# V-Sense/LFBM5D

Hardware: AMD Instinct MI355X
Metric: SAI-megapixels/sec (HT+Wiener, sigma=25) (higher is better)
Workload: dtype f32; 1 GPU; lf17x17x512x512_sigma25; light_field=17x17x512x512x3, asw=1, color_space=opp, noise=MT19937 seed 1 (utilities.cpp:176-183), window_lanes=2, spatial_bands=1, parallelism=single GPU

## Files before the change

### lfbm5d_amd/core.py

```python
import ctypes as C
import os
import subprocess

from typing import NamedTuple, Optional

import numpy as np

_HERE = os.path.dirname(os.path.abspath(__file__))

YUV, YCBCR, OPP, RGB, ID, DCT, SADCT, BIOR, HADAMARD, HAAR = range(10)
ROWMAJOR, COLMAJOR = 11, 12
TAU = {"id": ID, "dct": DCT, "sadct": SADCT, "bior": BIOR, "hw": HADAMARD, "haar": HAAR}
COLOR_SPACE = {"yuv": YUV, "ycbcr": YCBCR, "opp": OPP, "rgb": RGB}
UNIQUE_ID_BYTES = 128


class LfBm5dError(RuntimeError):
    pass


class Params(C.Structure):
    _fields_ = [("sigma", C.c_float), ("lambda_", C.c_float), ("N", C.c_uint), ("nSim", C.c_uint),
                ("nDisp", C.c_uint), ("k", C.c_uint), ("p", C.c_uint), ("useSD", C.c_uint),
                ("tau_2D", C.c_uint), ("tau_4D", C.c_uint), ("tau_5D", C.c_uint),
# ... 232 lines not shown
    out = (C.c_void_p * len(arrays))()
    for i, a in enumerate(arrays):
        if a is None or not mask[i]:
            continue
        if not (isinstance(a, np.ndarray) and a.dtype == np.float32 and a.flags.c_contiguous):
            raise LfBm5dError("per-SAI host buffers must be contiguous float32 numpy arrays")
        out[i] = a.ctypes.data
    return out


OPTION_ENV = ("LFBM5D_LANES", "LFBM5D_EMULATE_WORLD", "LFBM5D_MAX_WINDOWS", "LFBM5D_FUSED", "LFBM5D_STEP_SHARDING",
              "LFBM5D_DATA_DRIVEN_SCHEDULE", "LFBM5D_HOST_BLOCKING", "LFBM5D_BAND_MB", "LFBM5D_BM3D_LANES", "LFBM5D_SCAN_LDS_CAP",
              "LFBM5D_FORCE_REDO", "LFBM5D_SPATIAL_BANDS", "LFBM5D_BAND_HALO", "LFBM5D_SCAN_V1", "LFBM5D_SCAN_ANY", "LFBM5D_SCAN_FULL_TABLES", "LFBM5D_DCT8W_V2",
              "LFBM5D_GROUP_GENERIC", "LFBM5D_NO_SA_KERNELS", "LFBM5D_NO_SLAB_KERNEL", "LFBM5D_WIDE_NOSPLIT", "LFBM5D_AGG_64BIT",
              "LFBM5D_AGG_SCALAR_SCAN", "LFBM5D_SUBSET_LIST_HOST", "LFBM5D_SUBSET_SCAN_V1", "LFBM5D_FILT_GROUP_MAJOR",
              "LFBM5D_HT_REF_ORDER")


class Context:

    def __init__(self, device=0):
        self._L = lib()
        h = C.c_void_p()
        if self._L.lfbm5d_create(C.byref(h), int(device)) != 0:
            raise LfBm5dError(self._L.lfbm5d_last_error(None).decode())
        self._handle = h
        self._env_seen = {k: os.environ.get(k) for k in OPTION_ENV}
        self.device = int(device)

    @property
    def _h(self):
# ... 275 lines not shown
```

### lfbm5d_amd/csrc/lfbm5d_api.hip

```cpp
#include "lfbm5d_graph.h"

using namespace lfbm5d_host;
using lfbm5d::plan::search_window;
using lfbm5d::plan::plan_windows;

namespace { std::string g_create_error; }

extern "C" {

int lfbm5d_device_count(void) {
    int n = 0;
    if (hipGetDeviceCount(&n) != hipSuccess) return 0;
    return n;
}

int lfbm5d_create(lfbm5d_ctx** out, int device) {
    if (!out) return 1;
    *out = nullptr;
    int n = 0;
    hipError_t e = hipGetDeviceCount(&n);
    if (e != hipSuccess || n <= 0) {
        g_create_error = "no HIP device available (liblfbm5d_hip has no CPU fallback)";
        return 1;
    }
// ... 14 lines not shown
int lfbm5d_get_option(lfbm5d_ctx* c, const char* key, char* value, unsigned long long size) {
    if (!c || !key || !value || size == 0) return 1;
    std::string v;
    if (!option_get(c->opt_store, key, v)) return fail(c, std::string("unknown option: ") + key);
    std::snprintf(value, (size_t)size, "%s", v.c_str());
    return 0;
}

void lfbm5d_destroy(lfbm5d_ctx* c) {
    if (!c) return;
    (void)hipSetDevice(c->device);
    for (lfbm5d_ctx* x : c->lanes) lfbm5d_destroy(x);
    c->lanes.clear();
    if (c->h_counts) (void)hipHostFree(c->h_counts);
    if (c->stream) (void)hipStreamSynchronize(c->stream);
    for (lfbm5d_ctx::IpcPeer& P : c->ipc_peers) for (void* q : P.ptr) if (q) (void)hipIpcCloseMemHandle(q);
    c->ipc_flags.release(); c->ipc_out.release(); c->pristine.release(); c->pristine_b.release();
    if (c->io_in) (void)hipStreamDestroy(c->io_in);
    if (c->io_out) (void)hipStreamDestroy(c->io_out);
    if (c->team_comm2) ncclCommDestroy(c->team_comm2);
    if (c->team_comm) ncclCommDestroy(c->team_comm);
    if (c->comm2) ncclCommDestroy(c->comm2);
    if (c->comm) ncclCommDestroy(c->comm);
    for (int i = 0; i < 2; i++) if (c->cs[i]) (void)hipStreamDestroy(c->cs[i]);
    for (GeomCache& g : c->gc) { g.refs.release(); g.rslot.release(); g.tb.release(); g.scan_wgs.release(); }
    DevBuf* bufs[] = {&c->est, &c->g_num2, &c->g_den2, &c->n2, &c->e_basic, &c->refmap, &c->scores, &c->tables, &c->self_idx, &c->self_cnt, &c->best,
                      &c->t_noisy, &c->t_basic, &c->t_tnum, &c->t_tden, &c->und_num, &c->und_den, &c->sub_flags, &c->sub_cnt, &c->shape, &c->filt, &c->wgt, &c->aggpos, &c->gpos, &c->gofs, &c->gok, &c->sa_list, &c->gshape, &c->band_noisy, &c->band_basic, &c->band_out, &c->band_src, &c->band_pack, &c->band_gather, &c->counters, &c->small, &c->t_num, &c->t_den, &c->d_mask, &c->g_num, &c->g_den, &c->w_noisy,
                      &c->w_basic, &c->w_num, &c->w_den, &c->h2d_noisy, &c->h2d_basic, &c->h2d_out, &c->d_own, &c->gscratch, &c->scan_lcol};
    for (DevBuf* b : bufs) b->release();
    c->noise.sai.release(); c->noise.part.release(); c->noise.cells.release(); c->noise.m.release(); c->noise.pool.release();
    for (hipEvent_t e : c->ev_pool) (void)hipEventDestroy(e);
    if (c->h_small) (void)hipHostFree(c->h_small);
    if (c->stream) (void)hipStreamDestroy(c->stream);
    delete c;
}

const char* lfbm5d_last_error(const lfbm5d_ctx* c) { return c ? c->err.c_str() : g_create_error.c_str(); }
void lfbm5d_reset_stats(lfbm5d_ctx* c) { if (c) std::memset(&c->stats, 0, sizeof(c->stats)); }
void lfbm5d_get_stats(const lfbm5d_ctx* c, lfbm5d_stats* out) { if (c && out) *out = c->stats; }
void* lfbm5d_stream(lfbm5d_ctx* c) { return c ? (void*)c->stream : nullptr; }

void lfbm5d_shard_rows(unsigned n_rows, int rank, int world, unsigned* begin, unsigned* end) {
    if (world < 1) world = 1;
    if (rank < 0) rank = 0;
    *begin = (unsigned)(((unsigned long long)n_rows * (unsigned)rank) / (unsigned)world);
    *end = (unsigned)(((unsigned long long)n_rows * (unsigned)(rank + 1)) / (unsigned)world);
}
// ... 540 lines not shown
```

### lfbm5d_amd/csrc/lfbm5d_ctx.h

```cpp
#ifndef LFBM5D_CTX_H
#define LFBM5D_CTX_H

#include "../../include/lfbm5d.h"
#include "lfbm5d_kernels.h"
#include "lfbm5d_plan.h"
#include "lfbm5d_options.h"

#include <rccl/rccl.h>

#include <algorithm>
#include <chrono>
#include <cmath>
#include <fstream>
#include <thread>
#include <unistd.h>
#include <cstdio>
#include <cstdlib>
#include <cstring>
#include <string>
#include <vector>


namespace lfbm5d_host {

// ... 12 lines not shown
        if (p) { hipError_t e = hipFree(p); p = nullptr; cap = 0; if (e != hipSuccess) return e; }
        hipError_t e = hipMalloc(&p, bytes);
        if (e == hipSuccess) cap = bytes;
        return e;
    }
    void release() { if (p) (void)hipFree(p); p = nullptr; cap = 0; }
    template <class T> T* as() const { return reinterpret_cast<T*>(p); }
};

struct PassEvents { hipEvent_t e[5]; bool comm; };

struct GeomCache {
    DevBuf refs, rslot, tb, scan_wgs;
    std::vector<Scan2Wg> scan_plan; unsigned scan_key[8] = {0, 0, 0, 0, 0, 0, 0, 0}; size_t scan_lds = 0;
    unsigned scan_nwg_slot = 0; int scan_version = 0;
    std::vector<unsigned> last_refs_host;
    unsigned grid_key[5] = {0, 0, 0, 0, 0};
    unsigned rslot_key[5] = {0, 0, 0, 0, 0};
    unsigned tb_key[3] = {0, 0, 0};
    unsigned n_ref_rows = 0, n_ref_cols = 0;
};

}

using lfbm5d_host::DevBuf; using lfbm5d_host::PassEvents; using lfbm5d_host::GeomCache; using lfbm5d::Options;


constexpr int kDefaultLanes = 2;
constexpr size_t kEstLead = 64;

struct HostIO {
    float* const* noisy = nullptr;
    float* const* basic = nullptr;
    float* const* out = nullptr;
};

struct lfbm5d_ctx {
    int device = 0;
    hipStream_t stream = nullptr;
    std::string err;
    int rank = 0, world = 1;
    int tiles = 1;
    ncclComm_t comm = nullptr;
    ncclComm_t comm2 = nullptr;
    hipStream_t cs[2] = {nullptr, nullptr};
    int pass_rank = 0, pass_world = 1;
    bool pass_reduce = false;
    std::vector<unsigned> last_windows;
    lfbm5d_stats stats;
    DevBuf t_noisy, t_basic, t_tnum, t_tden, und_num, und_den;
    DevBuf scan_lcol;
    DevBuf sub_flags, sub_cnt;
    int last_scan_version = 0;
    GeomCache gc[2]; int gslot = 0;
// ... 69 lines not shown
```

### lfbm5d_amd/csrc/lfbm5d_graph.hip

```cpp
#include "lfbm5d_graph.h"

namespace lfbm5d_host {

using plan::search_window;
using plan::plan_windows;

int io_upload_all(lfbm5d_ctx* c, const HostIO* io, const unsigned* h_mask, unsigned asize, size_t img, float* d_noisy, float* d_basic_in) {
    for (unsigned st = 0; st < asize; st++) {
        if (!h_mask[st]) continue;
        HIPCK(c, hipMemcpyAsync(d_noisy + (size_t)st * img, io->noisy[st], img * sizeof(float), hipMemcpyHostToDevice, c->stream));
        if (d_basic_in) HIPCK(c, hipMemcpyAsync(d_basic_in + (size_t)st * img, io->basic[st], img * sizeof(float), hipMemcpyHostToDevice, c->stream));
    }
    HIPCK(c, hipStreamSynchronize(c->stream));
    return 0;
}
int io_download_all(lfbm5d_ctx* c, const HostIO* io, const unsigned* h_mask, unsigned asize, size_t img, const float* d_noisy,
                    const float* d_basic, const float* d_out) {
    for (unsigned st = 0; st < asize; st++) {
        if (!h_mask[st]) continue;
        HIPCK(c, hipMemcpyAsync(io->noisy[st], d_noisy + (size_t)st * img, img * sizeof(float), hipMemcpyDeviceToHost, c->stream));
        if (d_basic) HIPCK(c, hipMemcpyAsync(io->basic[st], d_basic + (size_t)st * img, img * sizeof(float), hipMemcpyDeviceToHost, c->stream));
        if (d_out) HIPCK(c, hipMemcpyAsync(io->out[st], d_out + (size_t)st * img, img * sizeof(float), hipMemcpyDeviceToHost, c->stream));
    }
    HIPCK(c, hipStreamSynchronize(c->stream));
// ... 295 lines not shown
            const unsigned cst_w = ang_major == LFBM5D_ROWMAJOR ? (unsigned)cs_w * g.asw + (unsigned)ct_w : (unsigned)cs_w + (unsigned)ct_w * g.asw;
            std::vector<unsigned> mask_w(g.Aw, 0), proc_w(g.Aw, 0);
            SaiList wl; wl.n = g.Aw;
            for (unsigned si = 0; si < g.asw; si++)
                for (unsigned ti = 0; ti < g.asw; ti++) {
                    const unsigned Ss = si + (unsigned)mins, T = ti + (unsigned)mint;
                    const unsigned st = ang_major == LFBM5D_ROWMAJOR ? Ss * awidth + T : Ss + T * aheight;
                    const unsigned slot = ang_major == LFBM5D_ROWMAJOR ? si * g.asw + ti : si + ti * g.asw;
                    mask_w[slot] = h_mask[st];
                    wl.st[slot] = h_mask[st] ? st : 0xffffffffu;
                    if (h_mask[st]) win_bits[n].set(slot);
                    proc_w[slot] = !h_mask[st];
                }
            const bool wien = J.step[sl] == 2;
            HIPCK(c, Lw.x->est.reserve((kEstLead + g.Aw * (size_t)g.wb * g.hb + 256) * sizeof(float)));
            HIPCK(c, launch_window_begin(ls, J.noisy[sl], wien ? S->basic : nullptr, S->g_num[sl], S->g_den[sl], img, Lw.w_noisy, Lw.w_basic, Lw.w_num,
                                         Lw.w_den, Lw.x->est.as<float>() + kEstLead, g.imgb, wl, W, H, C, g.nHW, Lw.d_small));
            lfbm5d_params Pw = *J.P[sl];
            Pw.tau_4D = nd.tau4;
            Lw.x->gslot = sl;
            Lw.x->est_ready = true;
            const int prc = pass_impl(Lw.x, J.step[sl], &Pw, g.asw, g.asw, g.wb, g.hb, C, Lw.w_noisy, wien ? Lw.w_basic : nullptr, Lw.w_num, Lw.w_den,
                                      mask_w.data(), proc_w.data(), cst_w, cst_w);
            Lw.x->gslot = 0;
            if (prc) { if (Lw.x != c) c->err = Lw.x->err; return 1; }
            HIPCK(c, launch_window_end(ls, S->g_num[sl], S->g_den[sl], img, Lw.w_num, Lw.w_den, g.imgb, wl, W, H, C, g.nHW, J.P[sl]->k, Lw.d_small));
            HIPCK(c, hipMemcpyAsync(c->h_counts + (size_t)n * kWinCounters, Lw.d_small, kWinCounters * sizeof(unsigned), hipMemcpyDeviceToHost, ls));
            if (!nd.fin.empty()) {
                SaiList fl; fl.n = 0;
                for (unsigned st : nd.fin) fl.st[fl.n++] = st;
                const bool colour = C == 3 && J.P[0]->color_space != LFBM5D_RGB;
                HIPCK(c, launch_finalize_multi(ls, S->g_num[0], S->g_den[0], J.noisy[0], S->basic, img, fl, J.P[0]->color_space, W * H, colour ? 1 : 0));
// ... 240 lines not shown
```

### lfbm5d_amd/csrc/lfbm5d_kernels.h

```cpp
#ifndef LFBM5D_KERNELS_H
#define LFBM5D_KERNELS_H

#include <hip/hip_runtime.h>
#include <vector>

#include "lfbm5d_options.h"

constexpr int kFiltStoreAux = 2;
constexpr int kFiltLoadAux = 0;

#if defined(__HIPCC__)
typedef float filt_v4f __attribute__((ext_vector_type(4)));
typedef float filt_v2f __attribute__((ext_vector_type(2)));
__device__ __forceinline__ void filt_put(float* p, const float v) { *p = v; }
__device__ __forceinline__ void filt_put2(filt_v2f* p, const filt_v2f v) { *p = v; }
__device__ __forceinline__ void filt_put4(filt_v4f* p, const filt_v4f v) { *p = v; }
__device__ __forceinline__ void filt_put4(float4* p, const float4 v) { *p = v; }
__device__ __forceinline__ void filt_put4_nt(filt_v4f* p, const filt_v4f v) { __builtin_nontemporal_store(v, p); }
#endif

namespace lfbm5d {

constexpr int kMaxK = 32;
constexpr int kMaxA = 49;
// ... 193 lines not shown
struct SaiList { unsigned st[kBigA]; unsigned n; };
hipError_t launch_finalize_multi(hipStream_t s, const float* num, const float* den, const float* sub, float* basic, size_t sai_stride,
                                 const SaiList& L, unsigned cs, unsigned n_px, int colour);
hipError_t launch_output_multi(hipStream_t s, const float* num, const float* den, const float* sub, float* out, float* basic,
                               const float* noisy_src, float* noisy_dst, size_t sai_stride, const SaiList& L, unsigned cs, unsigned n_px,
                               int colour);
hipError_t launch_ipc_set(hipStream_t s, unsigned* p, unsigned v);
hipError_t launch_ipc_wait(hipStream_t s, const unsigned* p, unsigned want, unsigned* err, double timeout_s);
hipError_t launch_symetrize_multi(hipStream_t s, const float* src, size_t src_stride, float* dst, size_t dst_stride,
                                  const SaiList& L, unsigned W, unsigned H, unsigned C, unsigned N);
hipError_t launch_unsymetrize_multi(hipStream_t s, float* dst, size_t dst_stride, const float* src, size_t src_stride,
                                    const SaiList& L, unsigned W, unsigned H, unsigned C, unsigned N);
constexpr unsigned kWinCounters = 32;
hipError_t launch_window_begin(hipStream_t s, const float* noisy, const float* basic, const float* num, const float* den, size_t lf_stride,
                               float* w_noisy, float* w_basic, float* w_num, float* w_den, float* est, size_t w_stride, const SaiList& L,
                               unsigned W, unsigned H, unsigned C, unsigned N, unsigned* zero);
hipError_t launch_window_end(hipStream_t s, float* num, float* den, size_t lf_stride, const float* w_num, const float* w_den, size_t w_stride,
                             const SaiList& L, unsigned W, unsigned H, unsigned C, unsigned N, unsigned k, unsigned* count);
hipError_t launch_estimate_multi(hipStream_t s, const float* num, const float* den, const float* sub, float* est,
                                 size_t plane, unsigned C, unsigned A, const SaiMask& mask_bits);
hipError_t launch_copy_rect(hipStream_t s, float* dst, size_t dst_stride, unsigned dW, unsigned dH, unsigned dx0, unsigned dy0,
                            const float* src, size_t src_stride, unsigned sW, unsigned sH, unsigned sx0, unsigned sy0,
                            unsigned w, unsigned h, unsigned C, unsigned n_slots, const SaiMask& mask_bits);
hipError_t launch_copy_rows(hipStream_t s, const float* src, unsigned src_H, unsigned src_row0, float* dst, unsigned dst_H, unsigned dst_row0,
                            unsigned n_rows, unsigned W, unsigned planes);
hipError_t launch_fill_f32(hipStream_t s, float* p, float v, size_t n);
hipError_t launch_fill_i32(hipStream_t s, int* p, int v, size_t n);
hipError_t launch_add(hipStream_t s, float* dst, const float* src, size_t n);
hipError_t launch_count_zeros(hipStream_t s, const float* den, size_t seg, unsigned n_seg,
                              unsigned* counts);
hipError_t launch_count_denoised(hipStream_t s, const float* den, size_t sai_stride, unsigned n_slots, const SaiMask& mask_bits,
                                 unsigned W, unsigned H, unsigned C, unsigned N, unsigned k, unsigned* count);
hipError_t launch_refmap(hipStream_t s, const unsigned* refs, unsigned n_refs, int* refmap);
hipError_t launch_subset_list(hipStream_t s, const float* den0, unsigned Wb, unsigned k, unsigned nHW, unsigned p, unsigned n_rows,
                              unsigned n_cols, unsigned last_r, unsigned last_c, unsigned char* flags, unsigned* refs, unsigned* count);
hipError_t launch_bm_scan(hipStream_t s, const ScanArgs& a);
int bm_scan_version(const ScanArgs& a);
bool scan2_plan(const ScanArgs& a, std::vector<Scan2Wg>& wgs, size_t* lds_bytes, unsigned* nwg_slot = nullptr);
size_t scan_tables_floats(const ScanArgs& a, int version, unsigned n_slots, unsigned nwg_slot);
unsigned scan2_lcol_stride(const ScanArgs& a);
hipError_t prepare_scan2_kernels();
hipError_t launch_bm_scan2(hipStream_t s, const ScanArgs& a, size_t lds_bytes, bool combined);
hipError_t launch_stereo_argmin3(hipStream_t s, const float* tables, const unsigned* st_of_slot, unsigned n_slots, unsigned nwg_slot,
                                 unsigned W, unsigned H, unsigned k, unsigned nDisp, float thr,
                                 unsigned* best, unsigned char* shape);
hipError_t launch_stereo_argmin2(hipStream_t s, const float* tables, const unsigned* st_of_slot, unsigned n_slots,
                                 unsigned W, unsigned H, unsigned k, unsigned nDisp, float thr,
                                 unsigned* best, unsigned char* shape);
hipError_t launch_self_select(hipStream_t s, const float* scores, const unsigned* refs, unsigned n_refs,
                              unsigned W, unsigned nSim, unsigned N, float thr, unsigned* self_idx,
                              unsigned* self_cnt,
                              unsigned grid_cols = 0, unsigned nHW = 0, unsigned p = 1, unsigned last_r = 0, unsigned last_c = 0);
hipError_t launch_self_trivial(hipStream_t s, const unsigned* refs, unsigned n_refs, unsigned* self_idx,
                               unsigned* self_cnt);
hipError_t launch_stereo_argmin(hipStream_t s, const float* tables, const unsigned* st_of_slot, unsigned n_slots,
                                unsigned W, unsigned H, unsigned k, unsigned nDisp, float thr,
                                unsigned* best, unsigned char* shape);
// ... 9 lines not shown
```

### lfbm5d_amd/csrc/lfbm5d_options.h

```cpp
#ifndef LFBM5D_OPTIONS_H
#define LFBM5D_OPTIONS_H

#include <cstddef>
#include <cstdlib>
#include <cstring>
#include <string>

namespace lfbm5d {

enum : unsigned {
    kOptScanV1 = 1u << 0,
    kOptScanAny = 1u << 1,
    kOptScanFullTables = 1u << 2,
    kOptDct8wV2 = 1u << 3,
    kOptGroupGeneric = 1u << 4,
    kOptNoSaKernels = 1u << 5,
    kOptNoSlabKernel = 1u << 6,
    kOptWideNoSplit = 1u << 7,
    kOptAgg64Bit = 1u << 8,
    kOptAggScalarScan = 1u << 9,
    kOptSubsetListHost = 1u << 10,
    kOptSubsetScanV1 = 1u << 11,
    kOptFiltGroupMajor = 1u << 12,
    kOptHtReferenceOrder = 1u << 13,
// ... 1 lines not shown

struct Options {
    int lanes = 2;
    int emulate_world = 0;
    int max_windows = 0;
    int fused = 1;
    int step_sharding = 0;
    int data_driven_schedule = 0;
    int host_blocking = 0;
    int band_mb = 0;
    int bm3d_lanes = 3;
    int scan_lds_cap = 0;
    int force_redo = 0;
    int spatial_bands = 1;
    int band_halo = 0;
    unsigned kernels = 0;
};

struct OptionKey { const char* key; const char* env; int Options::* field; unsigned bit; };

inline const OptionKey* option_keys(size_t* n) {
    static const OptionKey keys[] = {
        {"lanes", "LFBM5D_LANES", &Options::lanes, 0}, {"emulate_world", "LFBM5D_EMULATE_WORLD", &Options::emulate_world, 0},
        {"max_windows", "LFBM5D_MAX_WINDOWS", &Options::max_windows, 0}, {"fused", "LFBM5D_FUSED", &Options::fused, 0},
        {"step_sharding", "LFBM5D_STEP_SHARDING", &Options::step_sharding, 0},
        {"data_driven_schedule", "LFBM5D_DATA_DRIVEN_SCHEDULE", &Options::data_driven_schedule, 0},
        {"host_blocking", "LFBM5D_HOST_BLOCKING", &Options::host_blocking, 0}, {"band_mb", "LFBM5D_BAND_MB", &Options::band_mb, 0},
        {"bm3d_lanes", "LFBM5D_BM3D_LANES", &Options::bm3d_lanes, 0}, {"scan_lds_cap", "LFBM5D_SCAN_LDS_CAP", &Options::scan_lds_cap, 0},
        {"force_redo", "LFBM5D_FORCE_REDO", &Options::force_redo, 0}, {"spatial_bands", "LFBM5D_SPATIAL_BANDS", &Options::spatial_bands, 0},
        {"band_halo", "LFBM5D_BAND_HALO", &Options::band_halo, 0},
        {"scan_v1", "LFBM5D_SCAN_V1", nullptr, kOptScanV1}, {"scan_any", "LFBM5D_SCAN_ANY", nullptr, kOptScanAny},
        {"scan_full_tables", "LFBM5D_SCAN_FULL_TABLES", nullptr, kOptScanFullTables}, {"dct8w_v2", "LFBM5D_DCT8W_V2", nullptr, kOptDct8wV2},
        {"group_generic", "LFBM5D_GROUP_GENERIC", nullptr, kOptGroupGeneric}, {"no_sa_kernels", "LFBM5D_NO_SA_KERNELS", nullptr, kOptNoSaKernels},
        {"no_slab_kernel", "LFBM5D_NO_SLAB_KERNEL", nullptr, kOptNoSlabKernel}, {"wide_nosplit", "LFBM5D_WIDE_NOSPLIT", nullptr, kOptWideNoSplit},
        {"agg_64bit", "LFBM5D_AGG_64BIT", nullptr, kOptAgg64Bit}, {"agg_scalar_scan", "LFBM5D_AGG_SCALAR_SCAN", nullptr, kOptAggScalarScan},
        {"subset_list_host", "LFBM5D_SUBSET_LIST_HOST", nullptr, kOptSubsetListHost}, {"subset_scan_v1", "LFBM5D_SUBSET_SCAN_V1", nullptr, kOptSubsetScanV1},
        {"filt_group_major", "LFBM5D_FILT_GROUP_MAJOR", nullptr, kOptFiltGroupMajor},
        {"ht_reference_order", "LFBM5D_HT_REF_ORDER", nullptr, kOptHtReferenceOrder},
    };
    *n = sizeof(keys) / sizeof(keys[0]);
    return keys;
}

inline bool option_set(Options& o, const char* key, const char* value) {
    size_t n; const OptionKey* keys = option_keys(&n);
// ... 44 lines not shown
```

### lfbm5d_amd/csrc/lfbm5d_pass.hip

```cpp
#include "lfbm5d_ctx.h"

namespace lfbm5d_host {

lfbm5d_ctx* new_ctx(int device, std::string& err) {
    hipError_t e;
    lfbm5d_ctx* c = new lfbm5d_ctx();
    c->device = device;
    std::memset(&c->stats, 0, sizeof(c->stats));
    if ((e = hipStreamCreateWithFlags(&c->stream, hipStreamNonBlocking)) != hipSuccess) { err = hipGetErrorString(e); delete c; return nullptr; }
    if ((e = prepare_group_kernels()) != hipSuccess || (e = prepare_scan2_kernels()) != hipSuccess) { err = std::string("kernel LDS limits: ") + hipGetErrorString(e); (void)hipStreamDestroy(c->stream); delete c; return nullptr; }
    if ((e = hipHostMalloc((void**)&c->h_small, 64 * sizeof(unsigned))) != hipSuccess) { err = hipGetErrorString(e); (void)hipStreamDestroy(c->stream); delete c; return nullptr; }
    return c;
}


hipEvent_t get_event(lfbm5d_ctx* c) {
    if (c->ev_used == c->ev_pool.size()) {
        hipEvent_t e; (void)hipEventCreate(&e); c->ev_pool.push_back(e);
    }
    return c->ev_pool[c->ev_used++];
}

void drain_events(lfbm5d_ctx* c) {
    for (const PassEvents& pe : c->pending) {
        float ms = 0;
        if (hipEventElapsedTime(&ms, pe.e[0], pe.e[1]) == hipSuccess) c->stats.ms_bm += ms;
// ... 119 lines not shown
    if (P->tau_4D != LFBM5D_ID && P->tau_4D != LFBM5D_DCT && P->tau_4D != LFBM5D_SADCT) return fail(c, "bad tau_4D");
    if (P->tau_5D != LFBM5D_HAAR && P->tau_5D != LFBM5D_HADAMARD && P->tau_5D != LFBM5D_DCT) return fail(c, "bad tau_5D");
    if (!is_pow2(P->N) || P->N > (unsigned)kMaxN3) return fail(c, "unsupported: N must be a power of two <= 32");
    if (P->nSim < 1 || P->nDisp < 1 || P->p < 1) return fail(c, "bad search window / step");
    if (P->nSim > 48 || P->nDisp > 24) return fail(c, "unsupported: nSim > 48 or nDisp > 24");
    (void)step;
    return 0;
}

int pass_impl(lfbm5d_ctx* c, int step, const lfbm5d_params* P, unsigned aw, unsigned ah, unsigned Wb,
              unsigned Hb, unsigned C, const float* d_noisy, const float* d_basic, float* d_num,
              float* d_den, const unsigned* h_mask, const unsigned* h_proc, unsigned cst, unsigned pst,
              bool bm3d) {
    const bool est_ready = c->est_ready;
    c->est_ready = false;
    if (validate(c, step, P, aw, ah, C, bm3d)) return 1;
    if (step == 2 && !d_basic) return fail(c, "step 2 needs the basic estimate");
    const unsigned A = aw * ah, k = P->k, k2 = k * k, N = P->N, nHW = P->nSim + P->nDisp;
    const size_t plane = (size_t)Wb * Hb;
    hipStream_t s = c->stream;
    GeomCache& gc = c->gc[c->gslot];
    if (Hb < 2 * nHW + k + 1 || Wb < 2 * nHW + k + 1) return fail(c, "window smaller than the search range");
    if (Hb > 65535 || Wb > 65535) return fail(c, "unsupported: window larger than 65535 pixels a side");

    float sig[3] = {0, 0, 0};
    if (sigma_table(P->sigma, C, P->color_space, sig)) return fail(c, "bad color space");
    const float tauMatch = bm3d ? (step == 1 ? (C == 1 ? 3.f : 1.f) * (sig[0] < 35.0f ? 2500 : 5000)
                                             : (sig[0] < 35.0f ? 400.f : 3500.f))
                                : (C == 1 ? 3.f : 1.f) * (sig[0] < 35.0f ? (step == 1 ? 3000 : 2000) : 5000);
    const float thr = tauMatch * k * k;
// ... 145 lines not shown
        HIPCK(c, hipMemsetAsync(d_den, 0, A * C * plane * sizeof(float), s));
    }

    HIPCK(c, hipEventRecord(pe.e[0], s));
    ScanArgs sa;
    std::memset(&sa, 0, sizeof(sa));
    sa.dbg = d_counters + 4;
    sa.est = est; sa.W = Wb; sa.H = Hb; sa.k = k; sa.pst = pst;
    sa.nSim = P->nSim; sa.nDisp = P->nDisp; sa.nHW = nHW;
    sa.n_ref_rows = gc.n_ref_rows; sa.n_ref_cols = gc.n_ref_cols; sa.p = P->p;
    sa.scores = c->scores.as<float>(); sa.tables = c->tables.as<float>(); sa.rslot = gc.rslot.as<int>(); sa.refmap = (centre || full_scan) ? nullptr : c->refmap.as<int>(); sa.scores_bytes = (unsigned)((size_t)R_sc * NsS * NsS * sizeof(float));
    sa.n_self = N > 1 ? (P->nSim + 1) * NsS : 0;
    sa.n_stereo = n_slots * NsD * NsD;
    for (unsigned i = 0; i < n_slots; i++) sa.st_of_slot[i] = slots[i];
    sa.est_planes = A;
    if (N > 1) HIPCK(c, launch_fill_f32(s, c->scores.as<float>(), 2 * thr, (size_t)R_sc * NsS * NsS));
    sa.opt = c->opt->kernels; sa.lds_cap = (unsigned)std::max(0, c->opt->scan_lds_cap);
    const bool opt_v1 = (sa.opt & (kOptScanV1 | kOptScanAny)) != 0, opt_ft = (sa.opt & kOptScanFullTables) != 0;
    const unsigned skey[8] = {sa.n_self, sa.n_stereo, sa.nSim, sa.nDisp, sa.k, Hb, Wb,
                              1u | ((centre || full_scan) ? 0u : 2u) | (opt_v1 ? 4u : 0u) | (opt_ft ? 8u : 0u) | ((sa.opt & kOptScanAny) ? 16u : 0u)};
    const bool scan_changed = std::memcmp(skey, gc.scan_key, sizeof(skey)) != 0;
    if (scan_changed) gc.scan_version = bm_scan_version(sa);
    const int scan_version = gc.scan_version;
    c->last_scan_version = scan_version;
    if (scan_version == 1) {
        HIPCK(c, c->tables.reserve(std::max<size_t>(1, scan_tables_floats(sa, 1, n_slots, 0)) * sizeof(float)));
        sa.tables = c->tables.as<float>();
    }
    if (scan_version >= 2) {
        if (scan_changed) {
            if (!scan2_plan(sa, gc.scan_plan, &gc.scan_lds, &gc.scan_nwg_slot)) return fail(c, "scan plan");
            HIPCK(c, gc.scan_wgs.reserve(gc.scan_plan.size() * sizeof(Scan2Wg)));
            HIPCK(c, hipMemcpyAsync(gc.scan_wgs.p, gc.scan_plan.data(), gc.scan_plan.size() * sizeof(Scan2Wg), hipMemcpyHostToDevice, s));
            HIPCK(c, hipStreamSynchronize(s));
        }
        sa.wgs = gc.scan_wgs.as<Scan2Wg>(); sa.n_wgs = (unsigned)gc.scan_plan.size();
        sa.lcol_stride = scan2_lcol_stride(sa);
        HIPCK(c, c->scan_lcol.reserve((size_t)(sa.n_self + sa.n_stereo) * sa.lcol_stride * sizeof(float)));
        sa.lcol = c->scan_lcol.as<float>();
        sa.nwg_slot = gc.scan_nwg_slot;
        HIPCK(c, c->tables.reserve(std::max<size_t>(1, scan_tables_floats(sa, scan_version, n_slots, sa.nwg_slot)) * sizeof(float)));
        sa.tables = c->tables.as<float>();
        HIPCK(c, launch_bm_scan2(s, sa, gc.scan_lds, scan_version == 3));
    } else
        HIPCK(c, launch_bm_scan(s, sa));
    std::memcpy(gc.scan_key, skey, sizeof(skey));
    if (N > 1)
        HIPCK(c, launch_self_select(s, c->scores.as<float>(), gc.refs.as<unsigned>(), R, Wb, P->nSim, N, thr,
                                    c->self_idx.as<unsigned>(), c->self_cnt.as<unsigned>(),
                                    full_scan ? gc.n_ref_cols : 0u, nHW, P->p, Hb - k - nHW, Wb - k - nHW));
    else
        HIPCK(c, launch_self_trivial(s, gc.refs.as<unsigned>(), R, c->self_idx.as<unsigned>(), c->self_cnt.as<unsigned>()));
    if (n_slots && scan_version == 3)
        HIPCK(c, launch_stereo_argmin3(s, c->tables.as<float>(), slots, n_slots, sa.nwg_slot, Wb, Hb, k, P->nDisp, thr,
                                       c->best.as<unsigned>(), c->shape.as<unsigned char>()));
    else if (n_slots && scan_version == 2)
        HIPCK(c, launch_stereo_argmin2(s, c->tables.as<float>(), slots, n_slots, Wb, Hb, k, P->nDisp, thr,
                                       c->best.as<unsigned>(), c->shape.as<unsigned char>()));
    else if (n_slots)
        HIPCK(c, launch_stereo_argmin(s, c->tables.as<float>(), slots, n_slots, Wb, Hb, k, P->nDisp, thr,
                                      c->best.as<unsigned>(), c->shape.as<unsigned char>()));
    HIPCK(c, hipEventRecord(pe.e[1], s));

    unsigned ref_begin, n_groups;
    if (centre) {
        unsigned rb = 0, re = gc.n_ref_rows;
        lfbm5d_shard_rows(gc.n_ref_rows, c->pass_rank, c->pass_world, &rb, &re);
        ref_begin = rb * gc.n_ref_cols; n_groups = (re - rb) * gc.n_ref_cols;
    } else {
        unsigned rb = 0, re = (unsigned)row_start.size() - 1;
        lfbm5d_shard_rows((unsigned)row_start.size() - 1, c->pass_rank, c->pass_world, &rb, &re);
        ref_begin = row_start[rb]; n_groups = row_start[re] - row_start[rb];
    }

    GroupArgs ga;
    std::memset(&ga, 0, sizeof(ga));
// ... 109 lines not shown
```

### lfbm5d_amd/csrc/lfbm5d_scan2.hip

```cpp
#include "lfbm5d_kernels.h"

#include <algorithm>
#include <cstdlib>
#include <cstring>
#include <type_traits>
#include <vector>

#pragma clang fp contract(off)

namespace lfbm5d {

namespace {

typedef float v4f __attribute__((ext_vector_type(4)));
typedef int v4i __attribute__((ext_vector_type(4)));

constexpr unsigned kRsrcFlags = 0x00020000u;
constexpr int kPairStoreAux = 2;
constexpr int kS2HandAux = 17;
constexpr int kLeadBytes = 32;

template <int K> struct S2Geom {
    static constexpr int CW1 = 64 + K;
    static constexpr int LAG = (63 - K + 7) / 8;
// ... 698 lines not shown
unsigned scan2_lcol_stride(const ScanArgs& a) {
    const unsigned rows_self = a.n_self ? a.H - 2 * a.nHW : 0, rows_st = a.n_stereo ? a.H - 2 * a.nDisp - (a.k - 1) : 0;
    return ((std::max(rows_self, rows_st) + 64 + 160 + 63) / 64) * 64;
}

hipError_t prepare_scan2_kernels() {
    const void* fns[] = {reinterpret_cast<const void*>(&k_bm_scan2<8, false>), reinterpret_cast<const void*>(&k_bm_scan2<16, false>),
                         reinterpret_cast<const void*>(&k_bm_scan2<8, true>), reinterpret_cast<const void*>(&k_bm_scan2<16, true>)};
    for (const void* f : fns) {
        const hipError_t e = hipFuncSetAttribute(f, hipFuncAttributeMaxDynamicSharedMemorySize, 160 * 1024);
        if (e != hipSuccess) return e;
    }
    return hipSuccess;
}

hipError_t launch_bm_scan2(hipStream_t s, const ScanArgs& a, size_t lds, bool combined) {
    if (!a.n_wgs) return hipSuccess;
    const dim3 blk((kS2NW + kS2NL) * 64);
    if (a.k == 8 && combined) hipLaunchKernelGGL((k_bm_scan2<8, true>), dim3(a.n_wgs), blk, lds, s, a);
    else if (a.k == 8) hipLaunchKernelGGL((k_bm_scan2<8, false>), dim3(a.n_wgs), blk, lds, s, a);
    else if (a.k == 16 && combined) hipLaunchKernelGGL((k_bm_scan2<16, true>), dim3(a.n_wgs), blk, lds, s, a);
    else if (a.k == 16) hipLaunchKernelGGL((k_bm_scan2<16, false>), dim3(a.n_wgs), blk, lds, s, a);
    else return hipErrorInvalidValue;
    return hipGetLastError();
}

struct Argmin3Args { const float* tables; unsigned st_of_slot[kBigA]; int W, H, k, nDisp, n_slots, nwg_slot; float thr; unsigned* best; unsigned char* shape; };
__global__ __launch_bounds__(256) void k_stereo_argmin3(Argmin3Args a) {
    const int W = a.W, H = a.H, nDisp = a.nDisp;
    const int span_c = W - 2 * nDisp - a.k + 1, span_r = H - 2 * nDisp - a.k + 1;
    const int nstrips = (span_c - 1 + 63) / 64;
// ... 91 lines not shown
```

### lfbm5d_amd/csrc/lfbm5d_window.hip

```cpp
#include "lfbm5d_kernels.h"

#include <algorithm>

namespace lfbm5d {

namespace {


__device__ __forceinline__ void color_px(unsigned cs, int fwd, const float R, const float G, const float B, float& x, float& y, float& z) {
#pragma clang fp contract(off)
    if (cs == 0) {
        if (fwd) { x = 0.299f * R + 0.587f * G + 0.114f * B; y = -0.14713f * R - 0.28886f * G + 0.436f * B; z = 0.615f * R - 0.51498f * G - 0.10001f * B; }
        else     { x = R + 1.13983f * B; y = R - 0.39465f * G - 0.5806f * B; z = R + 2.03211f * G; }
    } else if (cs == 1) {
        if (fwd) { x = 0.299f * R + 0.587f * G + 0.114f * B; y = -0.169f * R - 0.331f * G + 0.500f * B; z = 0.500f * R - 0.419f * G - 0.081f * B; }
        else     { x = 1.000f * R + 0.000f * G + 1.402f * B; y = 1.000f * R - 0.344f * G - 0.714f * B; z = 1.000f * R + 1.772f * G + 0.000f * B; }
    } else {
        if (fwd) { x = 0.333f * R + 0.333f * G + 0.333f * B; y = 0.500f * R + 0.000f * G - 0.500f * B; z = 0.250f * R - 0.500f * G + 0.250f * B; }
        else     { x = 1.0f * R + 1.0f * G + 0.666f * B; y = 1.0f * R + 0.0f * G - 1.333f * B; z = 1.0f * R - 1.0f * G + 0.666f * B; }
    }
}

__global__ void k_color(float* __restrict__ img, size_t sai_stride, const unsigned* __restrict__ mask, unsigned cs, unsigned n, int fwd) {
    const unsigned i = blockIdx.x * blockDim.x + threadIdx.x;
// ... 218 lines not shown
        c += den[(size_t)ch * w * h + (size_t)(N + r / sw) * w + N + r % sw] > 0.0f ? 1u : 0u;
    }
    const unsigned t = block_sum_u32(c, red);
    if (threadIdx.x == 0 && t) atomicAdd(count, t);
}

struct WinBeginArgs {
    const float* noisy; const float* basic; const float* num; const float* den;
    float* w_noisy; float* w_basic; float* w_num; float* w_den;
    float* est;
    size_t lf_stride, w_stride;
    SaiList L;
    int W, H, C, N;
    unsigned* zero;
};
__global__ __launch_bounds__(256) void k_window_begin(WinBeginArgs a) {
    if (blockIdx.x == 0 && blockIdx.y == 0 && blockIdx.z == 0 && threadIdx.y == 0 && threadIdx.x < kWinCounters && a.zero) a.zero[threadIdx.x] = 0u;
    const unsigned st = a.L.st[blockIdx.z];
    if (st == 0xffffffffu) return;
    const int w = a.W + 2 * a.N, h = a.H + 2 * a.N;
    const int xx = blockIdx.x * 64 + threadIdx.x, yy = blockIdx.y * 4 + threadIdx.y;
    if (xx >= w || yy >= h) return;
    const size_t so = (size_t)st * a.lf_stride + (size_t)mirror(yy - a.N, a.H) * a.W + mirror(xx - a.N, a.W);
    const size_t d_o = (size_t)blockIdx.z * a.w_stride + (size_t)yy * w + xx;
    const size_t sp = (size_t)a.W * a.H, dp = (size_t)w * h;
    float n0 = 0.0f, u0 = 0.0f, d0 = 0.0f, b0 = 0.0f;
    for (int c = 0; c < a.C; c++) {
        const float nv = a.noisy[so + c * sp], uv = a.num[so + c * sp], dv = a.den[so + c * sp];
        a.w_noisy[d_o + c * dp] = nv; a.w_num[d_o + c * dp] = uv; a.w_den[d_o + c * dp] = dv;
        float bv = 0.0f;
        if (a.basic) { bv = a.basic[so + c * sp]; a.w_basic[d_o + c * dp] = bv; }
        if (c == 0) { n0 = nv; u0 = uv; d0 = dv; b0 = bv; }
    }
    a.est[(size_t)blockIdx.z * dp + (size_t)yy * w + xx] = d0 ? __fdiv_rn(u0, d0) : (a.basic ? b0 : n0);
}

struct WinEndArgs {
    float* num; float* den; const float* w_num; const float* w_den;
    size_t lf_stride, w_stride;
    SaiList L;
    int W, H, C, N, k;
    unsigned* count;
};
constexpr int kWinEndRows = 32;
static_assert(kWinCounters == 32, "k_window_end");
constexpr int kWinEndCounters = 32;
__global__ __launch_bounds__(256) void k_window_end(WinEndArgs a) {
    __shared__ unsigned red[4];
    const unsigned st = a.L.st[blockIdx.z];
// ... 92 lines not shown
}
hipError_t launch_symetrize_multi(hipStream_t s, const float* src, size_t src_stride, float* dst, size_t dst_stride,
                                  const SaiList& L, unsigned W, unsigned H, unsigned C, unsigned N) {
    hipLaunchKernelGGL(k_symetrize_multi, dim3(grid1d((size_t)(W + 2 * N) * (H + 2 * N) * C).x, L.n), dim3(256), 0, s,
                       src, src_stride, dst, dst_stride, L, (int)W, (int)H, (int)C, (int)N);
    return hipGetLastError();
}
hipError_t launch_unsymetrize_multi(hipStream_t s, float* dst, size_t dst_stride, const float* src, size_t src_stride,
                                    const SaiList& L, unsigned W, unsigned H, unsigned C, unsigned N) {
    hipLaunchKernelGGL(k_unsymetrize_multi, dim3(grid1d((size_t)W * H * C).x, L.n), dim3(256), 0, s,
                       dst, dst_stride, src, src_stride, L, (int)W, (int)H, (int)C, (int)N);
    return hipGetLastError();
}
hipError_t launch_window_begin(hipStream_t s, const float* noisy, const float* basic, const float* num, const float* den, size_t lf_stride,
                               float* w_noisy, float* w_basic, float* w_num, float* w_den, float* est, size_t w_stride, const SaiList& L,
                               unsigned W, unsigned H, unsigned C, unsigned N, unsigned* zero) {
    WinBeginArgs a;
    a.noisy = noisy; a.basic = basic; a.num = num; a.den = den; a.w_noisy = w_noisy; a.w_basic = w_basic; a.w_num = w_num; a.w_den = w_den;
    a.est = est; a.lf_stride = lf_stride; a.w_stride = w_stride; a.L = L; a.W = (int)W; a.H = (int)H; a.C = (int)C; a.N = (int)N; a.zero = zero;
    hipLaunchKernelGGL(k_window_begin, dim3((W + 2 * N + 63) / 64, (H + 2 * N + 3) / 4, L.n), dim3(64, 4), 0, s, a);
    return hipGetLastError();
}
hipError_t launch_window_end(hipStream_t s, float* num, float* den, size_t lf_stride, const float* w_num, const float* w_den, size_t w_stride,
                             const SaiList& L, unsigned W, unsigned H, unsigned C, unsigned N, unsigned k, unsigned* count) {
    WinEndArgs a;
    a.num = num; a.den = den; a.w_num = w_num; a.w_den = w_den; a.lf_stride = lf_stride; a.w_stride = w_stride; a.L = L;
    a.W = (int)W; a.H = (int)H; a.C = (int)C; a.N = (int)N; a.k = (int)k; a.count = count;
    hipLaunchKernelGGL(k_window_end, dim3((W + 63) / 64, (H + kWinEndRows - 1) / kWinEndRows, L.n), dim3(64, 4), 0, s, a);
    return hipGetLastError();
}
hipError_t launch_estimate_multi(hipStream_t s, const float* num, const float* den, const float* sub, float* est,
                                 size_t plane, unsigned C, unsigned A, const SaiMask& mask_bits) {
    hipLaunchKernelGGL(k_estimate_multi, dim3(grid1d(plane).x, A), dim3(256), 0, s, num, den, sub, est, plane, C, mask_bits);
    return hipGetLastError();
}
// ... 38 lines not shown
```

Baseline: 248.0 SAI-megapixels/s.

## Overlap window-begin copy and self-similarity scan on a side stream

Adds a second HIP stream per context. The window-begin kernel is split so that only the estimate part runs on the main stream while the window copies run on the side stream. The block-matching scan is also split: the self-similarity workgroups, the score fill and self-select run on the side stream while the stereo workgroups run on the main stream, joined by events. The goal is to let independent kernels run concurrently and fill the GPU better, at the cost of extra event and stream synchronisation overhead and some ordering risk.

```diff
diff --git a/lfbm5d_amd/core.py b/lfbm5d_amd/core.py
--- a/lfbm5d_amd/core.py
+++ b/lfbm5d_amd/core.py
@@ -270,7 +270,7 @@
               "LFBM5D_FORCE_REDO", "LFBM5D_SPATIAL_BANDS", "LFBM5D_BAND_HALO", "LFBM5D_SCAN_V1", "LFBM5D_SCAN_ANY", "LFBM5D_SCAN_FULL_TABLES", "LFBM5D_DCT8W_V2",
               "LFBM5D_GROUP_GENERIC", "LFBM5D_NO_SA_KERNELS", "LFBM5D_NO_SLAB_KERNEL", "LFBM5D_WIDE_NOSPLIT", "LFBM5D_AGG_64BIT",
               "LFBM5D_AGG_SCALAR_SCAN", "LFBM5D_SUBSET_LIST_HOST", "LFBM5D_SUBSET_SCAN_V1", "LFBM5D_FILT_GROUP_MAJOR",
-              "LFBM5D_HT_REF_ORDER")
+              "LFBM5D_HT_REF_ORDER", "LFBM5D_PASS_OVERLAP")
 
 
 class Context:
diff --git a/lfbm5d_amd/csrc/lfbm5d_api.hip b/lfbm5d_amd/csrc/lfbm5d_api.hip
--- a/lfbm5d_amd/csrc/lfbm5d_api.hip
+++ b/lfbm5d_amd/csrc/lfbm5d_api.hip
@@ -52,6 +52,7 @@
     c->lanes.clear();
     if (c->h_counts) (void)hipHostFree(c->h_counts);
     if (c->stream) (void)hipStreamSynchronize(c->stream);
+    if (c->side) (void)hipStreamSynchronize(c->side);
     for (lfbm5d_ctx::IpcPeer& P : c->ipc_peers) for (void* q : P.ptr) if (q) (void)hipIpcCloseMemHandle(q);
     c->ipc_flags.release(); c->ipc_out.release(); c->pristine.release(); c->pristine_b.release();
     if (c->io_in) (void)hipStreamDestroy(c->io_in);
@@ -69,6 +70,7 @@
     c->noise.sai.release(); c->noise.part.release(); c->noise.cells.release(); c->noise.m.release(); c->noise.pool.release();
     for (hipEvent_t e : c->ev_pool) (void)hipEventDestroy(e);
     if (c->h_small) (void)hipHostFree(c->h_small);
+    if (c->side) (void)hipStreamDestroy(c->side);
     if (c->stream) (void)hipStreamDestroy(c->stream);
     delete c;
 }
diff --git a/lfbm5d_amd/csrc/lfbm5d_ctx.h b/lfbm5d_amd/csrc/lfbm5d_ctx.h
--- a/lfbm5d_amd/csrc/lfbm5d_ctx.h
+++ b/lfbm5d_amd/csrc/lfbm5d_ctx.h
@@ -50,6 +50,7 @@
     DevBuf refs, rslot, tb, scan_wgs;
     std::vector<Scan2Wg> scan_plan; unsigned scan_key[8] = {0, 0, 0, 0, 0, 0, 0, 0}; size_t scan_lds = 0;
     unsigned scan_nwg_slot = 0; int scan_version = 0;
+    unsigned scan_n_self_wgs = 0;
     std::vector<unsigned> last_refs_host;
     unsigned grid_key[5] = {0, 0, 0, 0, 0};
     unsigned rslot_key[5] = {0, 0, 0, 0, 0};
@@ -74,6 +75,8 @@
 struct lfbm5d_ctx {
     int device = 0;
     hipStream_t stream = nullptr;
+    hipStream_t side = nullptr;
+    bool side_pending = false;
     std::string err;
     int rank = 0, world = 1;
     int tiles = 1;
diff --git a/lfbm5d_amd/csrc/lfbm5d_graph.hip b/lfbm5d_amd/csrc/lfbm5d_graph.hip
--- a/lfbm5d_amd/csrc/lfbm5d_graph.hip
+++ b/lfbm5d_amd/csrc/lfbm5d_graph.hip
@@ -333,8 +333,18 @@
                 }
             const bool wien = J.step[sl] == 2;
             HIPCK(c, Lw.x->est.reserve((kEstLead + g.Aw * (size_t)g.wb * g.hb + 256) * sizeof(float)));
-            HIPCK(c, launch_window_begin(ls, J.noisy[sl], wien ? S->basic : nullptr, S->g_num[sl], S->g_den[sl], img, Lw.w_noisy, Lw.w_basic, Lw.w_num,
-                                         Lw.w_den, Lw.x->est.as<float>() + kEstLead, g.imgb, wl, W, H, C, g.nHW, Lw.d_small));
+            if (c->opt->pass_overlap) {
+                hipEvent_t ev_win = get_event(c);
+                HIPCK(c, hipEventRecord(ev_win, ls));
+                HIPCK(c, hipStreamWaitEvent(Lw.x->side, ev_win, 0));
+                HIPCK(c, launch_window_begin(Lw.x->side, J.noisy[sl], wien ? S->basic : nullptr, S->g_num[sl], S->g_den[sl], img, Lw.w_noisy, Lw.w_basic,
+                                             Lw.w_num, Lw.w_den, nullptr, g.imgb, wl, W, H, C, g.nHW, nullptr, 2));
+                Lw.x->side_pending = true;
+                HIPCK(c, launch_window_begin(ls, J.noisy[sl], wien ? S->basic : nullptr, S->g_num[sl], S->g_den[sl], img, nullptr, nullptr, nullptr,
+                                             nullptr, Lw.x->est.as<float>() + kEstLead, g.imgb, wl, W, H, C, g.nHW, Lw.d_small, 1));
+            } else
+                HIPCK(c, launch_window_begin(ls, J.noisy[sl], wien ? S->basic : nullptr, S->g_num[sl], S->g_den[sl], img, Lw.w_noisy, Lw.w_basic, Lw.w_num,
+                                             Lw.w_den, Lw.x->est.as<float>() + kEstLead, g.imgb, wl, W, H, C, g.nHW, Lw.d_small));
             lfbm5d_params Pw = *J.P[sl];
             Pw.tau_4D = nd.tau4;
             Lw.x->gslot = sl;
diff --git a/lfbm5d_amd/csrc/lfbm5d_kernels.h b/lfbm5d_amd/csrc/lfbm5d_kernels.h
--- a/lfbm5d_amd/csrc/lfbm5d_kernels.h
+++ b/lfbm5d_amd/csrc/lfbm5d_kernels.h
@@ -231,7 +231,7 @@
 constexpr unsigned kWinCounters = 32;
 hipError_t launch_window_begin(hipStream_t s, const float* noisy, const float* basic, const float* num, const float* den, size_t lf_stride,
                                float* w_noisy, float* w_basic, float* w_num, float* w_den, float* est, size_t w_stride, const SaiList& L,
-                               unsigned W, unsigned H, unsigned C, unsigned N, unsigned* zero);
+                               unsigned W, unsigned H, unsigned C, unsigned N, unsigned* zero, int part = 0);
 hipError_t launch_window_end(hipStream_t s, float* num, float* den, size_t lf_stride, const float* w_num, const float* w_den, size_t w_stride,
                              const SaiList& L, unsigned W, unsigned H, unsigned C, unsigned N, unsigned k, unsigned* count);
 hipError_t launch_estimate_multi(hipStream_t s, const float* num, const float* den, const float* sub, float* est,
@@ -257,7 +257,7 @@
 size_t scan_tables_floats(const ScanArgs& a, int version, unsigned n_slots, unsigned nwg_slot);
 unsigned scan2_lcol_stride(const ScanArgs& a);
 hipError_t prepare_scan2_kernels();
-hipError_t launch_bm_scan2(hipStream_t s, const ScanArgs& a, size_t lds_bytes, bool combined);
+hipError_t launch_bm_scan2(hipStream_t s, const ScanArgs& a, size_t lds_bytes, bool combined, unsigned first = 0, unsigned count = 0);
 hipError_t launch_stereo_argmin3(hipStream_t s, const float* tables, const unsigned* st_of_slot, unsigned n_slots, unsigned nwg_slot,
                                  unsigned W, unsigned H, unsigned k, unsigned nDisp, float thr,
                                  unsigned* best, unsigned char* shape);
diff --git a/lfbm5d_amd/csrc/lfbm5d_options.h b/lfbm5d_amd/csrc/lfbm5d_options.h
--- a/lfbm5d_amd/csrc/lfbm5d_options.h
+++ b/lfbm5d_amd/csrc/lfbm5d_options.h
@@ -39,6 +39,7 @@
     int force_redo = 0;
     int spatial_bands = 1;
     int band_halo = 0;
+    int pass_overlap = 1;
     unsigned kernels = 0;
 };
 
@@ -53,7 +54,7 @@
         {"host_blocking", "LFBM5D_HOST_BLOCKING", &Options::host_blocking, 0}, {"band_mb", "LFBM5D_BAND_MB", &Options::band_mb, 0},
         {"bm3d_lanes", "LFBM5D_BM3D_LANES", &Options::bm3d_lanes, 0}, {"scan_lds_cap", "LFBM5D_SCAN_LDS_CAP", &Options::scan_lds_cap, 0},
         {"force_redo", "LFBM5D_FORCE_REDO", &Options::force_redo, 0}, {"spatial_bands", "LFBM5D_SPATIAL_BANDS", &Options::spatial_bands, 0},
-        {"band_halo", "LFBM5D_BAND_HALO", &Options::band_halo, 0},
+        {"band_halo", "LFBM5D_BAND_HALO", &Options::band_halo, 0}, {"pass_overlap", "LFBM5D_PASS_OVERLAP", &Options::pass_overlap, 0},
         {"scan_v1", "LFBM5D_SCAN_V1", nullptr, kOptScanV1}, {"scan_any", "LFBM5D_SCAN_ANY", nullptr, kOptScanAny},
         {"scan_full_tables", "LFBM5D_SCAN_FULL_TABLES", nullptr, kOptScanFullTables}, {"dct8w_v2", "LFBM5D_DCT8W_V2", nullptr, kOptDct8wV2},
         {"group_generic", "LFBM5D_GROUP_GENERIC", nullptr, kOptGroupGeneric}, {"no_sa_kernels", "LFBM5D_NO_SA_KERNELS", nullptr, kOptNoSaKernels},
diff --git a/lfbm5d_amd/csrc/lfbm5d_pass.hip b/lfbm5d_amd/csrc/lfbm5d_pass.hip
--- a/lfbm5d_amd/csrc/lfbm5d_pass.hip
+++ b/lfbm5d_amd/csrc/lfbm5d_pass.hip
@@ -8,8 +8,10 @@
     c->device = device;
     std::memset(&c->stats, 0, sizeof(c->stats));
     if ((e = hipStreamCreateWithFlags(&c->stream, hipStreamNonBlocking)) != hipSuccess) { err = hipGetErrorString(e); delete c; return nullptr; }
-    if ((e = prepare_group_kernels()) != hipSuccess || (e = prepare_scan2_kernels()) != hipSuccess) { err = std::string("kernel LDS limits: ") + hipGetErrorString(e); (void)hipStreamDestroy(c->stream); delete c; return nullptr; }
-    if ((e = hipHostMalloc((void**)&c->h_small, 64 * sizeof(unsigned))) != hipSuccess) { err = hipGetErrorString(e); (void)hipStreamDestroy(c->stream); delete c; return nullptr; }
+    if ((e = hipStreamCreateWithFlags(&c->side, hipStreamNonBlocking)) != hipSuccess) { err = hipGetErrorString(e); (void)hipStreamDestroy(c->stream); delete c; return nullptr; }
+    auto drop = [&]() { (void)hipStreamDestroy(c->side); (void)hipStreamDestroy(c->stream); delete c; };
+    if ((e = prepare_group_kernels()) != hipSuccess || (e = prepare_scan2_kernels()) != hipSuccess) { err = std::string("kernel LDS limits: ") + hipGetErrorString(e); drop(); return nullptr; }
+    if ((e = hipHostMalloc((void**)&c->h_small, 64 * sizeof(unsigned))) != hipSuccess) { err = hipGetErrorString(e); drop(); return nullptr; }
     return c;
 }
 
@@ -159,6 +161,8 @@
               bool bm3d) {
     const bool est_ready = c->est_ready;
     c->est_ready = false;
+    const bool side_pending = c->side_pending;
+    c->side_pending = false;
     if (validate(c, step, P, aw, ah, C, bm3d)) return 1;
     if (step == 2 && !d_basic) return fail(c, "step 2 needs the basic estimate");
     const unsigned A = aw * ah, k = P->k, k2 = k * k, N = P->N, nHW = P->nSim + P->nDisp;
@@ -334,7 +338,6 @@
     sa.n_stereo = n_slots * NsD * NsD;
     for (unsigned i = 0; i < n_slots; i++) sa.st_of_slot[i] = slots[i];
     sa.est_planes = A;
-    if (N > 1) HIPCK(c, launch_fill_f32(s, c->scores.as<float>(), 2 * thr, (size_t)R_sc * NsS * NsS));
     sa.opt = c->opt->kernels; sa.lds_cap = (unsigned)std::max(0, c->opt->scan_lds_cap);
     const bool opt_v1 = (sa.opt & (kOptScanV1 | kOptScanAny)) != 0, opt_ft = (sa.opt & kOptScanFullTables) != 0;
     const unsigned skey[8] = {sa.n_self, sa.n_stereo, sa.nSim, sa.nDisp, sa.k, Hb, Wb,
@@ -353,6 +356,8 @@
             HIPCK(c, gc.scan_wgs.reserve(gc.scan_plan.size() * sizeof(Scan2Wg)));
             HIPCK(c, hipMemcpyAsync(gc.scan_wgs.p, gc.scan_plan.data(), gc.scan_plan.size() * sizeof(Scan2Wg), hipMemcpyHostToDevice, s));
             HIPCK(c, hipStreamSynchronize(s));
+            gc.scan_n_self_wgs = 0;
+            while (gc.scan_n_self_wgs < gc.scan_plan.size() && gc.scan_plan[gc.scan_n_self_wgs].slot < 0) gc.scan_n_self_wgs++;
         }
         sa.wgs = gc.scan_wgs.as<Scan2Wg>(); sa.n_wgs = (unsigned)gc.scan_plan.size();
         sa.lcol_stride = scan2_lcol_stride(sa);
@@ -361,12 +366,24 @@
         sa.nwg_slot = gc.scan_nwg_slot;
         HIPCK(c, c->tables.reserve(std::max<size_t>(1, scan_tables_floats(sa, scan_version, n_slots, sa.nwg_slot)) * sizeof(float)));
         sa.tables = c->tables.as<float>();
+    }
+    std::memcpy(gc.scan_key, skey, sizeof(skey));
+    const bool overlap = c->opt->pass_overlap != 0;
+    const bool split = overlap && scan_version >= 2 && N > 1 && sa.n_self > 0 && sa.n_stereo > 0 &&
+                       gc.scan_n_self_wgs > 0 && gc.scan_n_self_wgs < sa.n_wgs;
+    const bool join = split || side_pending;
+    hipStream_t ss = split ? c->side : s;
+    if (join) HIPCK(c, hipStreamWaitEvent(c->side, pe.e[0], 0));
+    if (N > 1) HIPCK(c, launch_fill_f32(ss, c->scores.as<float>(), 2 * thr, (size_t)R_sc * NsS * NsS));
+    if (split) {
+        HIPCK(c, launch_bm_scan2(ss, sa, gc.scan_lds, scan_version == 3, 0, gc.scan_n_self_wgs));
+        HIPCK(c, launch_bm_scan2(s, sa, gc.scan_lds, scan_version == 3, gc.scan_n_self_wgs, sa.n_wgs - gc.scan_n_self_wgs));
+    } else if (scan_version >= 2)
         HIPCK(c, launch_bm_scan2(s, sa, gc.scan_lds, scan_version == 3));
-    } else
+    else
         HIPCK(c, launch_bm_scan(s, sa));
-    std::memcpy(gc.scan_key, skey, sizeof(skey));
     if (N > 1)
-        HIPCK(c, launch_self_select(s, c->scores.as<float>(), gc.refs.as<unsigned>(), R, Wb, P->nSim, N, thr,
+        HIPCK(c, launch_self_select(ss, c->scores.as<float>(), gc.refs.as<unsigned>(), R, Wb, P->nSim, N, thr,
                                     c->self_idx.as<unsigned>(), c->self_cnt.as<unsigned>(),
                                     full_scan ? gc.n_ref_cols : 0u, nHW, P->p, Hb - k - nHW, Wb - k - nHW));
     else
@@ -380,6 +397,11 @@
     else if (n_slots)
         HIPCK(c, launch_stereo_argmin(s, c->tables.as<float>(), slots, n_slots, Wb, Hb, k, P->nDisp, thr,
                                       c->best.as<unsigned>(), c->shape.as<unsigned char>()));
+    if (join) {
+        hipEvent_t ej = get_event(c);
+        HIPCK(c, hipEventRecord(ej, c->side));
+        HIPCK(c, hipStreamWaitEvent(s, ej, 0));
+    }
     HIPCK(c, hipEventRecord(pe.e[1], s));
 
     unsigned ref_begin, n_groups;
diff --git a/lfbm5d_amd/csrc/lfbm5d_scan2.hip b/lfbm5d_amd/csrc/lfbm5d_scan2.hip
--- a/lfbm5d_amd/csrc/lfbm5d_scan2.hip
+++ b/lfbm5d_amd/csrc/lfbm5d_scan2.hip
@@ -736,7 +736,10 @@
     return hipSuccess;
 }
 
-hipError_t launch_bm_scan2(hipStream_t s, const ScanArgs& a, size_t lds, bool combined) {
+hipError_t launch_bm_scan2(hipStream_t s, const ScanArgs& a0, size_t lds, bool combined, unsigned first, unsigned count) {
+    if (first > a0.n_wgs || count > a0.n_wgs - first) return hipErrorInvalidValue;
+    ScanArgs a = a0;
+    a.wgs = a0.wgs + first; a.n_wgs = count ? count : a0.n_wgs - first;
     if (!a.n_wgs) return hipSuccess;
     const dim3 blk((kS2NW + kS2NL) * 64);
     if (a.k == 8 && combined) hipLaunchKernelGGL((k_bm_scan2<8, true>), dim3(a.n_wgs), blk, lds, s, a);
diff --git a/lfbm5d_amd/csrc/lfbm5d_window.hip b/lfbm5d_amd/csrc/lfbm5d_window.hip
--- a/lfbm5d_amd/csrc/lfbm5d_window.hip
+++ b/lfbm5d_amd/csrc/lfbm5d_window.hip
@@ -256,8 +256,9 @@
     int W, H, C, N;
     unsigned* zero;
 };
+template <int PART>
 __global__ __launch_bounds__(256) void k_window_begin(WinBeginArgs a) {
-    if (blockIdx.x == 0 && blockIdx.y == 0 && blockIdx.z == 0 && threadIdx.y == 0 && threadIdx.x < kWinCounters && a.zero) a.zero[threadIdx.x] = 0u;
+    if (PART != 2 && blockIdx.x == 0 && blockIdx.y == 0 && blockIdx.z == 0 && threadIdx.y == 0 && threadIdx.x < kWinCounters && a.zero) a.zero[threadIdx.x] = 0u;
     const unsigned st = a.L.st[blockIdx.z];
     if (st == 0xffffffffu) return;
     const int w = a.W + 2 * a.N, h = a.H + 2 * a.N;
@@ -266,6 +267,12 @@
     const size_t so = (size_t)st * a.lf_stride + (size_t)mirror(yy - a.N, a.H) * a.W + mirror(xx - a.N, a.W);
     const size_t d_o = (size_t)blockIdx.z * a.w_stride + (size_t)yy * w + xx;
     const size_t sp = (size_t)a.W * a.H, dp = (size_t)w * h;
+    if (PART == 1) {
+        const float u0 = a.num[so], d0 = a.den[so];
+        const float s0 = a.basic ? a.basic[so] : a.noisy[so];
+        a.est[(size_t)blockIdx.z * dp + (size_t)yy * w + xx] = d0 ? __fdiv_rn(u0, d0) : s0;
+        return;
+    }
     float n0 = 0.0f, u0 = 0.0f, d0 = 0.0f, b0 = 0.0f;
     for (int c = 0; c < a.C; c++) {
         const float nv = a.noisy[so + c * sp], uv = a.num[so + c * sp], dv = a.den[so + c * sp];
@@ -274,7 +281,7 @@
         if (a.basic) { bv = a.basic[so + c * sp]; a.w_basic[d_o + c * dp] = bv; }
         if (c == 0) { n0 = nv; u0 = uv; d0 = dv; b0 = bv; }
     }
-    a.est[(size_t)blockIdx.z * dp + (size_t)yy * w + xx] = d0 ? __fdiv_rn(u0, d0) : (a.basic ? b0 : n0);
+    if (PART == 0) a.est[(size_t)blockIdx.z * dp + (size_t)yy * w + xx] = d0 ? __fdiv_rn(u0, d0) : (a.basic ? b0 : n0);
 }
 
 struct WinEndArgs {
@@ -397,11 +404,14 @@
 }
 hipError_t launch_window_begin(hipStream_t s, const float* noisy, const float* basic, const float* num, const float* den, size_t lf_stride,
                                float* w_noisy, float* w_basic, float* w_num, float* w_den, float* est, size_t w_stride, const SaiList& L,
-                               unsigned W, unsigned H, unsigned C, unsigned N, unsigned* zero) {
+                               unsigned W, unsigned H, unsigned C, unsigned N, unsigned* zero, int part) {
     WinBeginArgs a;
     a.noisy = noisy; a.basic = basic; a.num = num; a.den = den; a.w_noisy = w_noisy; a.w_basic = w_basic; a.w_num = w_num; a.w_den = w_den;
     a.est = est; a.lf_stride = lf_stride; a.w_stride = w_stride; a.L = L; a.W = (int)W; a.H = (int)H; a.C = (int)C; a.N = (int)N; a.zero = zero;
-    hipLaunchKernelGGL(k_window_begin, dim3((W + 2 * N + 63) / 64, (H + 2 * N + 3) / 4, L.n), dim3(64, 4), 0, s, a);
+    const dim3 grid((W + 2 * N + 63) / 64, (H + 2 * N + 3) / 4, L.n);
+    if (part == 1) hipLaunchKernelGGL(k_window_begin<1>, grid, dim3(64, 4), 0, s, a);
+    else if (part == 2) hipLaunchKernelGGL(k_window_begin<2>, grid, dim3(64, 4), 0, s, a);
+    else hipLaunchKernelGGL(k_window_begin<0>, grid, dim3(64, 4), 0, s, a);
     return hipGetLastError();
 }
 hipError_t launch_window_end(hipStream_t s, float* num, float* den, size_t lf_stride, const float* w_num, const float* w_den, size_t w_stride,
```

Result: slower. 240.0 SAI-megapixels/s (-3.2%).
